# hungdinhxuan/real-time-deepfake-speech-detection

Hardware: AMD Instinct MI355X
Metric: utterances/sec (4 s @ 16 kHz) (higher is better)
Workload: dtype fp16

## Files before the change

real-time-deepfake-speech-detection_amd/csrc/afx_posconv.hip:

```cpp
#include "afx_common.h"
#include "afx_kernels.h"

namespace afx {

namespace {
constexpr int PC_C = 1024, PC_CPG = 64, PC_TAPS = 128, PC_RING = 4, PC_NW = 8, PC_MAXT = 4;
}

template <class HT>
__global__ __launch_bounds__(64 * PC_NW) void posconv_kernel(PosConvArgs p) {
  typedef typename HT::T T;
  typedef typename HT::V8 V8;
  extern __shared__ __attribute__((aligned(16))) char smem[];
  const int tid = threadIdx.x, lane = tid & 63;
  const int wave = __builtin_amdgcn_readfirstlane(tid >> 6);
  const int l15 = lane & 15, kq = lane >> 4;
  const int rows = p.slab_rows;
  const int slab_bytes = rows * 128;
  char* ring = smem + 2 * slab_bytes;
  const unsigned lds_base = (unsigned)(size_t)smem;
  const int id = blockIdx.x, k2 = id >> 3;
  const int grp = (id & 7) * 2 + (k2 & 1), pair = k2 >> 1;
  const int u0 = pair * 2;
  const int nslot = u0 + 1 < p.B ? 2 : 1;
  const T* xp = (const T*)p.xpad;
  const T* wg = (const T*)p.W + (long)grp * PC_CPG * (PC_CPG * PC_TAPS);

  auto dma16 = [&](const T* src, unsigned off) {
    unsigned keep;
    const unsigned dst = __builtin_amdgcn_readfirstlane(lds_base + off);
    asm volatile("s_mov_b32 %0, m0\n\ts_mov_b32 m0, %2\n\ts_nop 0\n\tglobal_load_lds_dwordx4 %1, off\n\ts_mov_b32 m0, %0"
                 : "=&s"(keep) : "v"(src), "s"(dst) : "memory");
  };
  const int last_row = p.T + PC_TAPS - 1;
  for (int s = 0; s < nslot; ++s) {
    const T* xb = xp + (long)(u0 + s) * p.xpad_batch + grp * PC_CPG;
    for (int q = wave; q < rows / 8; q += PC_NW) {
      int row = q * 8 + (lane >> 3);
      const int c = (lane & 7) ^ (((row >> 1) & 3) << 1);
      row = row < last_row ? row : last_row;
      dma16(xb + (long)row * PC_C + c * 8, s * slab_bytes + q * 1024);
    }
  }
  auto issue_tap = [&](int j) {
    static_assert(PC_NW == 8, "one 8-row piece of the 64-row weight tile per wave");
    const int row = wave * 8 + (lane >> 3);
    const int c = (lane & 7) ^ ((row >> 1) & 7);
    dma16(wg + (long)row * (PC_CPG * PC_TAPS) + j * PC_CPG + c * 8, 2 * slab_bytes + (j & (PC_RING - 1)) * 8192 + wave * 1024);
  };
  issue_tap(0);
  issue_tap(1);
  issue_tap(2);

  const int nrt = (p.T + 15) >> 4, ntiles = nslot * nrt;
  int abase[PC_MAXT], aoff[PC_MAXT];
#pragma unroll
  for (int i = 0; i < PC_MAXT; ++i) {
    const int q = wave + PC_NW * i;
    const int slot = q >= nrt ? 1 : 0, rt = q - slot * nrt;
    abase[i] = rt * 16 + l15;
    aoff[i] = slot * slab_bytes;
  }
  f32x4 acc[PC_MAXT][4];
#pragma unroll
  for (int i = 0; i < PC_MAXT; ++i)
#pragma unroll
    for (int c = 0; c < 4; ++c) acc[i][c] = f32x4{0.f, 0.f, 0.f, 0.f};
  const int wsw = (l15 >> 1) & 7;
  const int woff[2] = {l15 * 128 + ((kq ^ wsw) * 16), l15 * 128 + (((4 + kq) ^ wsw) * 16)};

  for (int j = 0; j < PC_TAPS; ++j) {
    if (j + 2 < PC_TAPS) asm volatile("s_waitcnt vmcnt(2)" ::: "memory");
    else if (j + 1 < PC_TAPS) asm volatile("s_waitcnt vmcnt(1)" ::: "memory");
    else asm volatile("s_waitcnt vmcnt(0)" ::: "memory");
    __builtin_amdgcn_s_barrier();
    asm volatile("" ::: "memory");
    if (j + 3 < PC_TAPS) issue_tap(j + 3);
    const char* wb = ring + (j & (PC_RING - 1)) * 8192;
    V8 wf[4][2];
#pragma unroll
    for (int c = 0; c < 4; ++c)
#pragma unroll
      for (int ks = 0; ks < 2; ++ks) wf[c][ks] = *(const V8*)(wb + c * 2048 + woff[ks]);
#pragma unroll
    for (int i = 0; i < PC_MAXT; ++i) {
      if (wave + PC_NW * i < ntiles) {
        const int R = abase[i] + j;
        const int sw = ((R >> 1) & 3) << 1;
        const V8 a0 = *(const V8*)(smem + aoff[i] + R * 128 + ((kq ^ sw) * 16));
        const V8 a1 = *(const V8*)(smem + aoff[i] + R * 128 + (((4 + kq) ^ sw) * 16));
#pragma unroll
        for (int c = 0; c < 4; ++c) acc[i][c] = HT::mfma(wf[c][0], a0, acc[i][c]);
#pragma unroll
        for (int c = 0; c < 4; ++c) acc[i][c] = HT::mfma(wf[c][1], a1, acc[i][c]);
      }
    }
  }

#pragma unroll
  for (int i = 0; i < PC_MAXT; ++i) {
    const int q = wave + PC_NW * i;
    if (q >= ntiles) continue;
    const int slot = q >= nrt ? 1 : 0, rt = q - slot * nrt;
    const int t = rt * 16 + l15;
    if (t >= p.T) continue;
    float* xr = p.x + ((long)(u0 + slot) * p.T + t) * PC_C + grp * PC_CPG;
    f32x4 bv[4], rv[4];
#pragma unroll
    for (int c = 0; c < 4; ++c) {
      const int col = c * 16 + kq * 4;
      bv[c] = *(const f32x4*)(p.bias + grp * PC_CPG + col);
      rv[c] = *(const f32x4*)(xr + col);
    }
#pragma unroll
    for (int c = 0; c < 4; ++c) {
      const int col = c * 16 + kq * 4;
      *(f32x4*)(xr + col) = rv[c] + gelu_poly4(acc[i][c] + bv[c]);
    }
  }
}

const char* launch_posconv(const PosConvArgs& p_in, int dtype, hipStream_t s) {
  PosConvArgs p = p_in;
  if (dtype == DT_FP32) return "posconv: half-precision operands only (exact mode uses the fp32 GEMM)";
  if (p.B <= 0 || p.T <= 0 || 2 * ((p.T + 15) / 16) > PC_NW * PC_MAXT || p.T > 224) return "posconv: 1..224 frames";
  p.slab_rows = (p.T + PC_TAPS - 1 + 7) & ~7;
  const int lds = 2 * p.slab_rows * 128 + PC_RING * 8192;
  if (lds > 160 * 1024) return "posconv: slab does not fit the LDS";
  static LdsLimit lim[2];
  hipError_t e = hipSuccess;
  const int npair = (p.B + 1) / 2;
  dim3 grid(16 * npair);
  if (dtype == DT_BF16) {
    e = lim[0].ensure((const void*)posconv_kernel<BF16>, lds);
    if (e == hipSuccess) hipLaunchKernelGGL(posconv_kernel<BF16>, grid, dim3(64 * PC_NW), lds, s, p);
  } else {
    e = lim[1].ensure((const void*)posconv_kernel<FP16>, lds);
    if (e == hipSuccess) hipLaunchKernelGGL(posconv_kernel<FP16>, grid, dim3(64 * PC_NW), lds, s, p);
  }
  if (e == hipSuccess) e = hipGetLastError();
  return e == hipSuccess ? nullptr : hipGetErrorString(e);
}

}
```

Baseline: 13400.

## Deepen posconv weight prefetch ring and software-pipeline LDS fragment reads

Grows the weight tap ring from 4 to 8 slots, with 6 taps in flight instead of 3, so more global-to-LDS latency is hidden. The tap loop is rewritten to double-buffer the weight and activation register fragments. Each tap's LDS reads are issued while the previous MFMAs run, with sched_barrier hints to keep them interleaved. A compile-time tile count per wave replaces the runtime per-tile guard. The costs are more LDS per block, more registers from the duplicated fragments, and four extra template instantiations.

```diff
diff --git a/real-time-deepfake-speech-detection_amd/csrc/afx_posconv.hip b/real-time-deepfake-speech-detection_amd/csrc/afx_posconv.hip
--- a/real-time-deepfake-speech-detection_amd/csrc/afx_posconv.hip
+++ b/real-time-deepfake-speech-detection_amd/csrc/afx_posconv.hip
@@ -1,23 +1,111 @@
 #include "afx_common.h"
 #include "afx_kernels.h"
+#include <type_traits>
 
 namespace afx {
 
 namespace {
-constexpr int PC_C = 1024, PC_CPG = 64, PC_TAPS = 128, PC_RING = 4, PC_NW = 8, PC_MAXT = 4;
+constexpr int PC_C = 1024, PC_CPG = 64, PC_TAPS = 128, PC_NW = 8, PC_MAXT = 4;
+constexpr int PC_RING = 8, PC_AHEAD = 6;
+
+template <class T>
+__device__ __forceinline__ void pc_dma16(const T* src, unsigned dst_in) {
+  unsigned keep;
+  const unsigned dst = __builtin_amdgcn_readfirstlane(dst_in);
+  asm volatile("s_mov_b32 %0, m0\n\ts_mov_b32 m0, %2\n\ts_nop 0\n\tglobal_load_lds_dwordx4 %1, off\n\ts_mov_b32 m0, %0"
+               : "=&s"(keep) : "v"(src), "s"(dst) : "memory");
+}
+
+template <class T>
+__device__ __forceinline__ void pc_issue_tap(const T* wg, unsigned ring_lds, int wave, int lane, int j) {
+  static_assert(PC_NW == 8, "one 8-row piece of the 64-row weight tile per wave");
+  const int row = wave * 8 + (lane >> 3);
+  const int c = (lane & 7) ^ ((row >> 1) & 7);
+  pc_dma16(wg + (long)row * (PC_CPG * PC_TAPS) + j * PC_CPG + c * 8, ring_lds + (j & (PC_RING - 1)) * 8192 + wave * 1024);
+}
+
+template <class HT, int NT>
+__device__ __forceinline__ void posconv_taps(char* smem, const typename HT::T* wg, unsigned lds_base, int slab_bytes, int nrt,
+                                             int wave, int lane, f32x4 (&acc)[PC_MAXT][4]) {
+  typedef typename HT::V8 V8;
+  const int l15 = lane & 15, kq = lane >> 4;
+  const unsigned ring_lds = lds_base + 2 * slab_bytes;
+  const char* ring = smem + 2 * slab_bytes;
+  constexpr int ND = NT > 0 ? NT : 1;
+  int arow[ND];
+#pragma unroll
+  for (int i = 0; i < NT; ++i) {
+    const int q = wave + PC_NW * i;
+    const int slot = q >= nrt ? 1 : 0, rt = q - slot * nrt;
+    arow[i] = slot * slab_bytes + (rt * 16 + l15) * 128;
+  }
+  const int wsw = (l15 >> 1) & 7;
+  const int woff[2] = {l15 * 128 + ((kq ^ wsw) * 16), l15 * 128 + (((4 + kq) ^ wsw) * 16)};
+  auto read_a = [&](V8 (&a)[2], int i, int j) {
+    const int sw = (((l15 + j) >> 1) & 3) << 1;
+    const char* r = smem + arow[i] + j * 128;
+    a[0] = *(const V8*)(r + ((kq ^ sw) * 16));
+    a[1] = *(const V8*)(r + (((4 + kq) ^ sw) * 16));
+  };
+  auto read_w = [&](V8 (&w)[4][2], int j, int n) {
+    w[n >> 1][n & 1] = *(const V8*)(ring + (j & (PC_RING - 1)) * 8192 + (n >> 1) * 2048 + woff[n & 1]);
+  };
+  V8 wf[2][4][2], af[2][2];
+  if (NT > 0) {
+#pragma unroll
+    for (int n = 0; n < 8; ++n) read_w(wf[0], 0, n);
+    read_a(af[0], 0, 0);
+  }
+  auto tap = [&](int t, auto H, auto W, auto ISSUE) {
+    constexpr int h = decltype(H)::value, w = decltype(W)::value;
+    asm volatile("s_waitcnt vmcnt(%0)" ::"n"(w) : "memory");
+    __builtin_amdgcn_s_barrier();
+    asm volatile("" ::: "memory");
+    if (decltype(ISSUE)::value) pc_issue_tap(wg, ring_lds, wave, lane, t + PC_AHEAD);
+    const int tn = (t + 1) & (PC_TAPS - 1);
+#pragma unroll
+    for (int i = 0; i < NT; ++i) {
+      const int cur = (h * NT + i) & 1;
+      if (i + 1 < NT) read_a(af[cur ^ 1], i + 1, t);
+      else read_a(af[cur ^ 1], 0, tn);
+#pragma unroll
+      for (int n = 8 * i / ND; n < 8 * (i + 1) / ND; ++n) read_w(wf[h ^ 1], tn, n);
+      __builtin_amdgcn_sched_barrier(0x6);
+#pragma unroll
+      for (int c = 0; c < 4; ++c) acc[i][c] = HT::mfma(wf[h][c][0], af[cur][0], acc[i][c]);
+#pragma unroll
+      for (int c = 0; c < 4; ++c) acc[i][c] = HT::mfma(wf[h][c][1], af[cur][1], acc[i][c]);
+    }
+  };
+  typedef std::integral_constant<int, 0> I0;
+  typedef std::integral_constant<int, 1> I1;
+  typedef std::integral_constant<int, 2> I2;
+  typedef std::integral_constant<int, 3> I3;
+  typedef std::integral_constant<int, 4> I4;
+  static_assert(PC_AHEAD == 6 && PC_TAPS % 2 == 0, "the tail below is written out for six taps ahead");
+  constexpr int steady = PC_TAPS - PC_AHEAD;
+  for (int j = 0; j < steady; j += 2) {
+    tap(j, I0(), I4(), I1());
+    tap(j + 1, I1(), I4(), I1());
+  }
+  tap(steady, I0(), I4(), I0());
+  tap(steady + 1, I1(), I3(), I0());
+  tap(steady + 2, I0(), I2(), I0());
+  tap(steady + 3, I1(), I1(), I0());
+  tap(steady + 4, I0(), I0(), I0());
+  tap(steady + 5, I1(), I0(), I0());
+}
 }
 
 template <class HT>
 __global__ __launch_bounds__(64 * PC_NW) void posconv_kernel(PosConvArgs p) {
   typedef typename HT::T T;
-  typedef typename HT::V8 V8;
   extern __shared__ __attribute__((aligned(16))) char smem[];
   const int tid = threadIdx.x, lane = tid & 63;
   const int wave = __builtin_amdgcn_readfirstlane(tid >> 6);
   const int l15 = lane & 15, kq = lane >> 4;
   const int rows = p.slab_rows;
   const int slab_bytes = rows * 128;
-  char* ring = smem + 2 * slab_bytes;
   const unsigned lds_base = (unsigned)(size_t)smem;
   const int id = blockIdx.x, k2 = id >> 3;
   const int grp = (id & 7) * 2 + (k2 & 1), pair = k2 >> 1;
@@ -26,12 +114,7 @@
   const T* xp = (const T*)p.xpad;
   const T* wg = (const T*)p.W + (long)grp * PC_CPG * (PC_CPG * PC_TAPS);
 
-  auto dma16 = [&](const T* src, unsigned off) {
-    unsigned keep;
-    const unsigned dst = __builtin_amdgcn_readfirstlane(lds_base + off);
-    asm volatile("s_mov_b32 %0, m0\n\ts_mov_b32 m0, %2\n\ts_nop 0\n\tglobal_load_lds_dwordx4 %1, off\n\ts_mov_b32 m0, %0"
-                 : "=&s"(keep) : "v"(src), "s"(dst) : "memory");
-  };
+  auto dma16 = [&](const T* src, unsigned off) { pc_dma16(src, lds_base + off); };
   const int last_row = p.T + PC_TAPS - 1;
   for (int s = 0; s < nslot; ++s) {
     const T* xb = xp + (long)(u0 + s) * p.xpad_batch + grp * PC_CPG;
@@ -42,59 +125,24 @@
       dma16(xb + (long)row * PC_C + c * 8, s * slab_bytes + q * 1024);
     }
   }
-  auto issue_tap = [&](int j) {
-    static_assert(PC_NW == 8, "one 8-row piece of the 64-row weight tile per wave");
-    const int row = wave * 8 + (lane >> 3);
-    const int c = (lane & 7) ^ ((row >> 1) & 7);
-    dma16(wg + (long)row * (PC_CPG * PC_TAPS) + j * PC_CPG + c * 8, 2 * slab_bytes + (j & (PC_RING - 1)) * 8192 + wave * 1024);
-  };
-  issue_tap(0);
-  issue_tap(1);
-  issue_tap(2);
+#pragma unroll
+  for (int j = 0; j < PC_AHEAD; ++j) pc_issue_tap(wg, lds_base + 2 * slab_bytes, wave, lane, j);
 
   const int nrt = (p.T + 15) >> 4, ntiles = nslot * nrt;
-  int abase[PC_MAXT], aoff[PC_MAXT];
-#pragma unroll
-  for (int i = 0; i < PC_MAXT; ++i) {
-    const int q = wave + PC_NW * i;
-    const int slot = q >= nrt ? 1 : 0, rt = q - slot * nrt;
-    abase[i] = rt * 16 + l15;
-    aoff[i] = slot * slab_bytes;
-  }
   f32x4 acc[PC_MAXT][4];
 #pragma unroll
   for (int i = 0; i < PC_MAXT; ++i)
 #pragma unroll
     for (int c = 0; c < 4; ++c) acc[i][c] = f32x4{0.f, 0.f, 0.f, 0.f};
-  const int wsw = (l15 >> 1) & 7;
-  const int woff[2] = {l15 * 128 + ((kq ^ wsw) * 16), l15 * 128 + (((4 + kq) ^ wsw) * 16)};
-
-  for (int j = 0; j < PC_TAPS; ++j) {
-    if (j + 2 < PC_TAPS) asm volatile("s_waitcnt vmcnt(2)" ::: "memory");
-    else if (j + 1 < PC_TAPS) asm volatile("s_waitcnt vmcnt(1)" ::: "memory");
-    else asm volatile("s_waitcnt vmcnt(0)" ::: "memory");
-    __builtin_amdgcn_s_barrier();
-    asm volatile("" ::: "memory");
-    if (j + 3 < PC_TAPS) issue_tap(j + 3);
-    const char* wb = ring + (j & (PC_RING - 1)) * 8192;
-    V8 wf[4][2];
-#pragma unroll
-    for (int c = 0; c < 4; ++c)
-#pragma unroll
-      for (int ks = 0; ks < 2; ++ks) wf[c][ks] = *(const V8*)(wb + c * 2048 + woff[ks]);
-#pragma unroll
-    for (int i = 0; i < PC_MAXT; ++i) {
-      if (wave + PC_NW * i < ntiles) {
-        const int R = abase[i] + j;
-        const int sw = ((R >> 1) & 3) << 1;
-        const V8 a0 = *(const V8*)(smem + aoff[i] + R * 128 + ((kq ^ sw) * 16));
-        const V8 a1 = *(const V8*)(smem + aoff[i] + R * 128 + (((4 + kq) ^ sw) * 16));
-#pragma unroll
-        for (int c = 0; c < 4; ++c) acc[i][c] = HT::mfma(wf[c][0], a0, acc[i][c]);
-#pragma unroll
-        for (int c = 0; c < 4; ++c) acc[i][c] = HT::mfma(wf[c][1], a1, acc[i][c]);
-      }
-    }
+  asm volatile("s_waitcnt vmcnt(5)" ::: "memory");
+  __builtin_amdgcn_s_barrier();
+  asm volatile("" ::: "memory");
+  switch (ntiles > wave ? (ntiles - wave + PC_NW - 1) / PC_NW : 0) {
+    case 0: posconv_taps<HT, 0>(smem, wg, lds_base, slab_bytes, nrt, wave, lane, acc); break;
+    case 1: posconv_taps<HT, 1>(smem, wg, lds_base, slab_bytes, nrt, wave, lane, acc); break;
+    case 2: posconv_taps<HT, 2>(smem, wg, lds_base, slab_bytes, nrt, wave, lane, acc); break;
+    case 3: posconv_taps<HT, 3>(smem, wg, lds_base, slab_bytes, nrt, wave, lane, acc); break;
+    default: posconv_taps<HT, 4>(smem, wg, lds_base, slab_bytes, nrt, wave, lane, acc); break;
   }
 
 #pragma unroll
```

Measured after the change: 13440 (median of 2 runs). No clear change (+0.3%).
